# UniBwTAS/continuous_clustering

Hardware: AMD Instinct MI355X
Metric: Mpoints/s clustered (64-beam streams) (higher is better)
Workload: dtype f32

## Files before the change

continuous_clustering_amd/csrc/cc_assoc3.h:

```cpp
#pragma once

constexpr int A3_REC = 8;
constexpr int A3_THREADS = 256;
constexpr int A3_PSTAGE = 8;
constexpr int A3_BIRTH = 8;

template<int RPL>
__device__ __forceinline__ void assoc3_stream(const Geometry& g, const cc_config& cfg, const Planes& P, StreamState* states, const int s, const int slot,
                                              const int limited)
{
    constexpr int G = RPL == 1 ? 8 : 4;
    constexpr int A2_LEAD = a2_lead(RPL), A2_STAGE = a2_stage(RPL);
    static_assert(WIN_COLS + A2_LEAD + 1 <= WIN2_COLS && A2_LEAD + G <= A2_STAGE && A2_LEAD < A2_INFO, "ring sizes");
    const int lane = lane_id();
    const int wave = uniform_i32((int) (threadIdx.x >> 6));
    const bool lwave = blockDim.x > 192;
    const int nthreads = (int) blockDim.x;
    StreamState* st = &states[s];
    if (st->error != 0 || st->batch[slot].seg_begin < 0 || st->assoc_mode != 0 || st->batch[slot].mode != 0 ||
        st->batch[slot].acp_next >= st->batch[slot].seg_end)
        return;
    AssocCtx c;
    c.p = stream_ptrs(P, g, s);
    const SP& p = c.p;
// ... 1297 lines not shown
                    }
                }
                wave_lds_fence();
            }

            A2_PH(3)
#ifdef CC_A2_STATS
            st_nunf += n_unf;
            st_sub++;
            st_check += cut == CUT_CHECK;
            st_live += cut == CUT_LIVE;
#endif
            int check_u = -1;
            if (cut == CUT_CHECK)
            {
                check_u = u1 - 1;
                u0 = u1;
            }
            else if (cut == CUT_LIVE)
            {
                const int u = u1;
                const long long gcu = gc + u;
                int lcu = lc0 + u;
                lcu = lcu >= RC ? lcu - RC : lcu;
                emit(CC_EV_GROUND_COLUMN, gcu, gcu, 0, 0, gcu);
                serial_cols++;
                wait_a(gcu + 1);
                if (err)
                    break;
                const int info_head = uniform_i32(lds_ld(&T.info_head[(int) (gcu & (A2_INFO - 1))]));
                park_a();
                if (err)
                    break;
                if (lane == 0)
                {
                    int nn = n_unf, e = 0, hd = info_head;
                    double LL = L;
                    long long MM = M;
                    assoc_column_live2<RPL>(c, cfg, g, T, s_win, lcu, gcu, (int) (first_unpub % RC), nn, LL, MM, hd, e, st);
                    T.bcast_i[0] = nn;
                    T.bcast_i[1] = e;
                    T.bcast_i[3] = hd;
                    T.bcast_d[0] = LL;
                    T.bcast_l[0] = MM;
                }
                wave_lds_fence();
                n_unf = uniform_i32(T.bcast_i[0]);
                const int hd = uniform_i32(T.bcast_i[3]);
                if (uniform_i32(T.bcast_i[1]) == CC_ERR_CAPACITY)
                {
                    err = CC_ERR_CAPACITY;
                    err_a = n_unf;
                }
                L = uniform_f64(T.bcast_d[0]);
                M = uniform_i64(T.bcast_l[0]);
                wave_lds_fence();
                if (err)
                    break;
                resume_a(gcu + 1, hd);
                check_u = u;
                u0 = u1 + 1;
                ids_stale = true;
            }
            else if (cut == CUT_GLOBAL)
            {
                to_global = true;
                gc += u1;
                break;
            }
            else
                u0 = gcount;
            if (check_u >= 0)
            {
                finish_and_publish(gc + check_u, lane_f64(v_minaz, check_u));
                verify |= killed;
            }
            if (lane == 0)
                lds_st(&T.b_done, gc + u0);
            A2_PH(4)
        }
        if (to_global || err)
            break;
        gc += gcount;
        lc0 += gcount;
        lc0 = lc0 >= RC ? lc0 - RC : lc0;
    }
    if (lane == 0)
        lds_st(&T.cmd, (int) A2_EXIT);
#ifdef CC_A2_STATS
    if (lane == 0)
    {
        st->dbg[8] += st_sub;
        st->dbg[9] += st_check;
        st->dbg[10] += __builtin_amdgcn_s_memtime() - st_t0;
        st->dbg[11] += st_live;
        st->dbg[12] += (unsigned long long) (gc - col_begin);
        st->dbg[13] += st_wait_g;
        st->dbg[14] += st_full;
        st->dbg[15] += st_kill;
        for (int i = 0; i < 5; i++)
            st->dbg[i] += st_ph[i];
    }
#endif

    {
        wave_lds_fence();
        for (int r = lane; r < n_unf; r += 64)
        {
            const int i = T.alist[r];
            const int cell = T.cell[i];
            p.ulist[r] = cell;
            p.t_pos[cell] = r;
            p.t_fin[cell] = __longlong_as_double((long long) T.fin[i]);
            p.t_width[cell] = (unsigned) (T.last[i] - T.gcol[i] + 1);
            p.t_pts[cell] = T.pts[i];
            p.t_uf[cell] = T.cell[T.uf[i]];
            p.t_cid[cell] = 0;
            p.t_finished[cell] = 0;
        }
    }
    if (lane == 0)
    {
        st->first_unpublished = first_unpub;
        st->batch[slot].pub_end = first_unpub;
        st->ring_start = ring_start;
        st->cluster_counter = cluster_counter;
        st->n_unfinished = n_unf;
        st->min_required = M;
        st->finish_lower_bound = L;
        st->last_round_min_az = last_min_az;
        st->cells_published = cells_published;
        st->clusters_finished = clusters_finished;
        st->exceed_one_rotation = exceed;
        st->serial_columns = serial_cols;
        st->stamp_alias_rounds = alias_rounds;
        st->batch[slot].acp_next = gc;
        st->n_events = n_events < g.event_capacity ? n_events : g.event_capacity;
        if (g.record_events && n_events > g.event_capacity && err == 0)
        {
            err = CC_ERR_CAPACITY;
            err_a = n_events;
        }
        if (to_global)
            st->assoc_mode = 1;
        if (err)
            raise_error(st, err, err_a, err_b);
    }
}

template<int RPL>
__global__ __launch_bounds__(A3_THREADS) void k_assoc3(Geometry g, cc_config cfg, Planes P, StreamState* states, int first_stream, int slot,
                                                       int limited, int count, int with_global)
{
    if (gridDim.x >= (unsigned) count)
    {
        if ((int) blockIdx.x < count)
        {
            assoc3_stream<RPL>(g, cfg, P, states, first_stream + (int) blockIdx.x, slot, limited);
            if (with_global && !limited)
            {
                __threadfence_block();
                __syncthreads();
                if (threadIdx.x < 64)
                    associate_stream<RPL>(g, cfg, P, states, first_stream + (int) blockIdx.x, slot);
            }
        }
        return;
    }
    __shared__ int s_work[A3_THREADS];
    __shared__ int s_nwork;
    if (threadIdx.x == 0)
        s_nwork = 0;
    __syncthreads();
    for (int base = 0; base < count; base += (int) (gridDim.x * blockDim.x))
    {
        const int i = base + (int) threadIdx.x * (int) gridDim.x + (int) blockIdx.x;
        if (i < count)
        {
            const StreamState* st = &states[first_stream + i];
            if (st->error == 0 && st->batch[slot].seg_begin >= 0 && st->batch[slot].acp_next < st->batch[slot].seg_end)
                s_work[atomicAdd(&s_nwork, 1)] = i;
        }
        __syncthreads();
        const int nw = s_nwork;
        for (int k = 0; k < nw; k++)
        {
            assoc3_stream<RPL>(g, cfg, P, states, first_stream + s_work[k], slot, limited);
            __threadfence_block();
            __syncthreads();
            if (with_global && !limited)
            {
                if (threadIdx.x < 64)
                    associate_stream<RPL>(g, cfg, P, states, first_stream + s_work[k], slot);
                __syncthreads();
            }
        }
        if (threadIdx.x == 0)
            s_nwork = 0;
        __syncthreads();
    }
}
```

continuous_clustering_amd/csrc/cc_engine.hip:

```cpp
#include <hip/hip_runtime.h>

#include <algorithm>
#include <chrono>
#include <cstdlib>
#include <cmath>
#include <cstdio>
#include <cstring>
#include <functional>
#include <limits>
#include <mutex>
#include <string>
#include <vector>

#include "cc_kernels.h"

#ifndef CC_LWAVE_MAX_STREAMS
#define CC_LWAVE_MAX_STREAMS 256
#endif

using namespace ccd;

struct cc_engine
{
    int device{0};
    Geometry g{};
    cc_config cfg{};
    Planes P{};
    StreamState* d_states{nullptr};
    int* d_remaining{nullptr};
    int* h_remaining{nullptr};
    int* d_bail_count{nullptr};
    int* h_bail_count{nullptr};
    int bail_seen{0}, bail_cooldown{0};
    int chronic_seen{0}, chronic_skip{0};
    bool chronic_probe{false};
    int assoc_sweep_blocks{2};
    int bail_cooldown_batches{4};
    bool capturing{false};
    cck::HostMirror capture_mirror{nullptr, nullptr, 0, nullptr, nullptr, nullptr, nullptr};
    int* d_par_left{nullptr};
    bool small_front{true};
    bool small_all{true};
    bool small_direct{true};
    int seg_small_max{63};
    bool fuse_front{true};
    int* h_par_left{nullptr};
    int insert_split_blocks{0};
    int insert_wide_max_streams{160};
    bool skip_idle_fallbacks{true};
    hipStream_t stream{nullptr};
    hipStream_t stream2{nullptr};
    hipStream_t stream3{nullptr};
    hipStream_t stream4{nullptr};
    hipStream_t stream6{nullptr};
    hipEvent_t ev_pubrdy[4]{};
    hipStream_t stream5{nullptr};
    hipEvent_t ev_ins[4]{}, ev_seg[4]{}, ev_assoc[4]{}, ev_segscan[4]{}, ev_prep[4]{};
    hipEvent_t ev_input{};
    int pipeline_depth{2};
    int prep_buf{0};
    std::vector<hipEvent_t> pev_pool;
    size_t pev_used{0};
    struct PrepPlanes
    {
        float *x, *y, *z, *dist, *incl, *incaz;
        int32_t* cir;
    } pp[2]{};
    uint64_t batch_seq{0};
    static constexpr int REL_RING = 8;
    uint64_t call_seq{0};
    uint64_t released_seq{0};
    hipEvent_t ev_rel[REL_RING]{};
    uint64_t rel_recorded[REL_RING]{};
    bool in_submit{false};
    bool cur_call_last{true};
    int check_input_lifetime{0};
    struct InputRec
    {
        uint64_t seq;
        const void *xyz, *inten, *pose;
        size_t b_xyz, b_int, b_pose;
        unsigned long long sum;
    };
    std::vector<InputRec> live_inputs;
    unsigned long long* d_input_sum{nullptr};
    unsigned long long* h_input_sum{nullptr};
    bool pipelined{false};
    bool allow_pipeline{true};
    bool host_prof{false};
    double hp_pre{0}, hp_gate{0}, hp_post{0}, hp_entry{0};
    long long hp_calls{0};
    bool parallel_insert_multi{true};
    bool parallel_insert{true};
    struct SmallGraph
    {
        int stream;
        int64_t n;
        int record;
        hipGraphExec_t exec;
    };
    std::vector<SmallGraph> small_graphs;
    unsigned char* h_small{nullptr};
    unsigned char* d_small{nullptr};
    unsigned long long* h_small_seq{nullptr};
    unsigned long long* d_small_seq{nullptr};
    unsigned long long small_seq_expected{0};
    unsigned long long small_tail_launches{0};
    long long* h_small_view_hdr{nullptr};
    char* h_small_view{nullptr};
    bool small_view_ok{false};
    int small_view_stream{-1};
    bool mirror_views{true};
    unsigned long long view_hits{0}, view_misses{0};
    bool resident_opt{false};
    bool res_running{false};
    cck::ResidentCtl* h_res_ctl{nullptr};
    int res_idle_ms{20};
    unsigned long long res_launches{0}, res_calls{0};
    StreamState* h_small_state{nullptr};
    cc_event* h_small_events{nullptr};
    bool allow_graphs{true};
    int scan_store_fin{-1};
    int scan_split{2};
    bool split_on{false};
    unsigned split_cols_seen{0}, split_rec_seen{0}, split_probe{0};
    int scan_packed{-1};
    int assoc_waves{3};
    bool assoc_batch{true};
    int assoc_rounds{0};
    bool assoc_waves_auto{true};
    bool assoc_pending[4]{false, false, false, false};
    std::vector<void*> allocations;
    std::function<int(const std::function<int()>*)> deferred_tail;
    int lazy_gate_max_streams{40};
    int lazy_gate_from_streams{80};
    bool lazy_ok{true};
    bool lazy_pending{false};
    const int* lazy_prev_left{nullptr};
    int lazy_miss{0};
    int lazy_clean{0};
    uint64_t lazy_batches{0}, lazy_redone{0};
    hipEvent_t ev_gate[4]{};
    int defer_tail_max_streams{96};
    bool slab_planning{false};
    size_t slab_bytes{0};
    std::vector<std::pair<void**, size_t>> slab_plan;
    std::string error;
    float* d_stage_xyz{nullptr};
    uint8_t* d_stage_int{nullptr};
    double* d_stage_pose{nullptr};
    int64_t stage_capacity{0};
    size_t prep_capacity{0};
    void* d_view{nullptr};
    size_t view_bytes{0};
    double* d_ego[4]{nullptr, nullptr, nullptr, nullptr};
    size_t ego_capacity{0};
    bool small_graphs_stale{false};
    bool idle{false};
    std::vector<StreamState> state_cache;
    std::vector<char> state_cached;
    char* d_gather{nullptr};
    size_t gather_bytes{0};
    char* h_view{nullptr};
    size_t h_view_bytes{0};
    std::vector<std::vector<cc_event>> pending_events;
    std::vector<std::vector<int64_t>> pending_links;
    const float* last_xyz{nullptr};
    const uint8_t* last_int{nullptr};
    const double* last_pose{nullptr};
    int64_t last_n{0};
    int64_t cur_ntotal{0}, cur_f0{0};
    int64_t sub_batch{0};
    bool input_on_engine_stream{false};
    int last_first{0}, last_count{0};
    bool batch_open{false};
    bool timing{false};
    int timing_every{1};
    uint64_t timing_pass{0};
    double prep_ahead_ms{0};
    std::vector<hipEvent_t> ev_pool;
    size_t ev_used{0};
    double kernel_ms[7]{0, 0, 0, 0, 0, 0, 0};
    uint64_t kernel_launches{0};
};

namespace
{

constexpr size_t CC_SLAB_ALIGN = 2u << 20;

#define CC_HIP_CHECK(e, call)                                                                                      \
    do                                                                                                             \
    {                                                                                                              \
        hipError_t _err = (call);                                                                                  \
        if (_err != hipSuccess)                                                                                    \
        {                                                                                                          \
            (e)->error = std::string(#call) + ": " + hipGetErrorString(_err);                                      \
            return CC_ERR_HIP;                                                                                     \
        }                                                                                                          \
    } while (0)

template<class T>
int alloc_plane(cc_engine* e, T** out, size_t count)
{
    if (e->slab_planning)
    {
        const size_t bytes = (count * sizeof(T) + CC_SLAB_ALIGN - 1) / CC_SLAB_ALIGN * CC_SLAB_ALIGN;
        e->slab_plan.push_back({(void**) out, e->slab_bytes});
        e->slab_bytes += bytes;
        return CC_OK;
    }
    void* p = nullptr;
    hipError_t err = hipMalloc(&p, count * sizeof(T));
    if (err != hipSuccess)
    {
        e->error = std::string("hipMalloc: ") + hipGetErrorString(err);
        return CC_ERR_HIP;
    }
    e->allocations.push_back(p);
    *out = (T*) p;
    return CC_OK;
}

int validate(cc_engine* e, const cc_config* cfg, int num_rows, int num_streams)
{
    if (!cfg || num_rows < 1 || num_rows > WAVE * MAX_ROWS_PER_LANE || num_streams < 1 || cfg->num_columns < 4 ||
        cfg->cluster_point_trees_every_nth_column < 1)
    {
        if (e)
            e->error = "invalid argument (num_rows must be 1..128, num_columns >= 4, every_nth_column >= 1)";
        return CC_ERR_INVALID_ARGUMENT;
    }
    return CC_OK;
}

void fill_geometry(cc_engine* e, int num_rows)
{
    Geometry& g = e->g;
    g.num_rows = num_rows;
    g.num_columns = e->cfg.num_columns;
    g.az_width = static_cast<float>((2 * M_PI)) / static_cast<float>(g.num_columns);
    g.ring_cols = g.num_columns * 10;
    g.cells = (int64_t) g.ring_cols * num_rows;
    g.max_distance_squared = e->cfg.max_distance * e->cfg.max_distance;
    g.limit_columns = 2 * g.num_columns;
    g.tab_tiles = g.ring_cols / 64 + 2;
    if (g.lds_tree_limit <= 0 || g.lds_tree_limit > TREE_SLOTS)
        g.lds_tree_limit = TREE_SLOTS;
    if (g.sl_cap <= 0 || g.sl_cap > cck::SL_CAP)
        g.sl_cap = cck::SL_CAP;
    if (g.scan_cap <= 0)
        g.scan_cap = cck::SCAN_CAP;
    g.scan_stores_fin = 0;
}

int free_all(cc_engine* e)
{
    for (void* p : e->allocations)
        (void) hipFree(p);
    e->allocations.clear();
    e->d_stage_xyz = nullptr;
    e->d_stage_int = nullptr;
    e->d_stage_pose = nullptr;
    e->stage_capacity = 0;
    e->d_view = nullptr;
    e->view_bytes = 0;
    e->prep_capacity = 0;
    e->ego_capacity = 0;
    e->d_gather = nullptr;
    e->gather_bytes = 0;
    e->d_small = nullptr;
    e->d_small_seq = nullptr;
    e->d_input_sum = nullptr;
    if (e->h_res_ctl)
        (void) hipHostFree(e->h_res_ctl);
    e->h_res_ctl = nullptr;
    if (e->h_small_view_hdr)
        (void) hipHostFree(e->h_small_view_hdr);
    if (e->h_small_view)
        (void) hipHostFree(e->h_small_view);
    e->h_small_view_hdr = nullptr;
    e->h_small_view = nullptr;
    e->small_view_ok = false;
    if (e->h_input_sum)
        (void) hipHostFree(e->h_input_sum);
    e->h_input_sum = nullptr;
    e->small_seq_expected = 0;
    if (e->h_small)
    {
        (void) hipHostFree(e->h_small);
        (void) hipHostFree(e->h_small_state);
        (void) hipHostFree(e->h_small_events);
        if (e->h_small_seq)
            (void) hipHostFree(e->h_small_seq);
        e->h_small_seq = nullptr;
        e->h_small = nullptr;
        e->h_small_state = nullptr;
        e->h_small_events = nullptr;
    }
    return CC_OK;
}

int allocate(cc_engine* e)
{
    const Geometry& g = e->g;
    const size_t S = (size_t) g.num_streams;
    const size_t C = S * (size_t) g.cells;
    const size_t L = S * (size_t) g.ring_cols;
    const size_t T = S * (size_t) g.tree_capacity;
    Planes& P = e->P;
    int rc = CC_OK;
    e->slab_planning = getenv("CC_NO_SLAB") == nullptr;
    e->slab_bytes = 0;
    e->slab_plan.clear();
#define A(field, count)                                \
    if ((rc = alloc_plane(e, &P.field, (count))) != 0) \
        return rc;
    A(dist, C) A(incl, C) A(incaz, C) A(gtag, C) A(src, C) A(inten, C);
    A(trig, L) A(colg, L) A(colminaz, L);
    A(ground, C) A(debug, C) A(ignored, C) A(root, C) A(id, C);
    A(t_fin, C) A(t_width, C) A(t_pts, C) A(t_uf, C) A(t_cid, C) A(t_pos, C) A(t_finished, C);
    A(ulist, T) A(ucomp, T) A(agg_fin, T) A(agg_min, T) A(agg_max, T) A(agg_pts, T) A(agg_cid, T) A(agg_first, T) A(agg_flag, T);
    A(events, S * (size_t) g.event_capacity);
    A(sc_parent, C) A(sc_nlinks, C) A(sc_links, C) A(sc_fin, C);
    A(sc_term, C) A(col_newfin, L) A(col_info, L) A(col_act, L) A(pk_meta, C) A(pk_fin, C) A(pk_lk, C);
    A(sg_x2, C) A(sg_uz, C) A(sg_w, C) A(sg_flags, C) A(sc_rec, C);
    A(curtab, S * (size_t) g.num_rows);
    A(tab_acc, S * (size_t) g.tab_tiles * (size_t) g.num_rows);
    A(par_off, S * (size_t) cck::IP_MAXF);
    A(tabc, (size_t) BATCH_SLOTS * S * (size_t) g.tab_tiles * (size_t) g.num_rows);
    A(sc_visits, C);
    A(link_log, S * (size_t) g.link_capacity);
    A(sl_ctl, S * 4) A(sl_cols, L);
    if ((rc = alloc_plane(e, (unsigned long long**) &P.sl_rec, S * (size_t) cck::SL_CAP * sizeof(cck::ScanLongRec) / sizeof(unsigned long long))) != 0)
        return rc;
#undef A
    if ((rc = alloc_plane(e, &e->d_states, S)) != 0)
        return rc;
    if ((rc = alloc_plane(e, &e->d_par_left, 16)) != 0)
        return rc;
    if ((rc = alloc_plane(e, &e->d_bail_count, 4)) != 0)
        return rc;
    if ((rc = alloc_plane(e, &e->d_remaining, 1)) != 0)
        return rc;
    const bool slab = e->slab_planning;
    if (e->slab_planning)
    {
        e->slab_planning = false;
        char* base = nullptr;
        if ((rc = alloc_plane(e, &base, e->slab_bytes)) != 0)
            return rc;
        for (auto& f : e->slab_plan)
            *f.first = base + f.second;
        e->slab_plan.clear();
    }
    (void) slab;
    CC_HIP_CHECK(e, hipMemset(e->d_bail_count, 0, 4 * sizeof(int)));
    CC_HIP_CHECK(e, hipMemset(e->d_par_left, 0, 16 * sizeof(int)));
    CC_HIP_CHECK(e, hipMemset(e->d_remaining, 0, sizeof(int)));
    return CC_OK;
}

int reset_state(cc_engine* e, bool keep_table)
{
    e->small_view_ok = false;
    std::fill(e->state_cached.begin(), e->state_cached.end(), 0);
    const Geometry& g = e->g;
    const size_t S = (size_t) g.num_streams;
    const size_t C = S * (size_t) g.cells;
    Planes& P = e->P;
    CC_HIP_CHECK(e, hipMemsetAsync(P.dist, 0xFF, C * sizeof(float), e->stream));
    CC_HIP_CHECK(e, hipMemsetAsync(P.incl, 0xFF, C * sizeof(float), e->stream));
    CC_HIP_CHECK(e, hipMemsetAsync(P.gtag, 0, C * sizeof(uint16_t), e->stream));
    CC_HIP_CHECK(e, hipMemsetAsync(P.id, 0, C * sizeof(uint32_t), e->stream));
    CC_HIP_CHECK(e, hipMemsetAsync(P.ground, CC_GP_UNKNOWN, C, e->stream));
    CC_HIP_CHECK(e, hipMemsetAsync(P.debug, CC_DBG_WHITE, C, e->stream));
    CC_HIP_CHECK(e, hipMemsetAsync(P.ignored, 0, C, e->stream));
    CC_HIP_CHECK(e, hipMemsetAsync(P.root, 0xFF, C * sizeof(int32_t), e->stream));
    CC_HIP_CHECK(e, hipMemsetAsync(P.tab_acc, 0, S * (size_t) g.tab_tiles * (size_t) g.num_rows * sizeof(unsigned long long), e->stream));
    CC_HIP_CHECK(e, hipMemsetAsync(P.sl_ctl, 0, S * 4 * sizeof(int32_t), e->stream));
    if (!keep_table)
        CC_HIP_CHECK(e, hipMemsetAsync(P.curtab, 0xFF, S * (size_t) g.num_rows * sizeof(float), e->stream));
    std::vector<StreamState> init(S);
    for (auto& st : init)
    {
        memset(&st, 0, sizeof(st));
        st.prev_rearmost = 0;
        st.prev_foremost = -1;
        st.first_unfinished = -1;
        st.ring_start = -1;
        st.ring_end = -1;
        st.first_column = -1;
        st.clear_done = -1;
        st.first_unpublished = -1;
        st.cluster_counter = 1;
        st.min_required = 0;
        st.finish_lower_bound = std::numeric_limits<double>::max();
        st.last_round_min_az = -1.0;
        st.overrun_col = std::numeric_limits<int64_t>::max();
        st.n_links = 0;
        for (auto& d : st.batch)
            d.seg_begin = d.seg_end = d.acp_next = d.pub_begin = d.pub_end = -1, d.mode = 0, d.fused = 0;
        st.assoc_mode = e->cfg.max_steps_in_row > WIN_COLS - 2 ? 1 : 0;
    }
    CC_HIP_CHECK(e, hipMemcpyAsync(e->d_states, init.data(), S * sizeof(StreamState), hipMemcpyHostToDevice, e->stream));
    CC_HIP_CHECK(e, hipStreamSynchronize(e->stream));
    for (auto& v : e->pending_events)
        v.clear();
    for (auto& v : e->pending_links)
        v.clear();
    e->batch_open = false;
    for (bool& b : e->assoc_pending)
        b = false;
    e->deferred_tail = nullptr;
    e->lazy_pending = false;
    e->lazy_prev_left = nullptr;
    e->lazy_miss = 0;
    e->lazy_clean = 0;
    e->lazy_ok = true;
    return CC_OK;
}

int ensure_prep(cc_engine* e, size_t points)
{
    if (e->prep_capacity >= points)
        return CC_OK;
    int rc;
    for (auto& q : e->pp)
        if ((rc = alloc_plane(e, &q.x, points)) || (rc = alloc_plane(e, &q.y, points)) || (rc = alloc_plane(e, &q.z, points)) ||
            (rc = alloc_plane(e, &q.dist, points)) || (rc = alloc_plane(e, &q.incl, points)) ||
            (rc = alloc_plane(e, &q.incaz, points)) || (rc = alloc_plane(e, &q.cir, points)))
            return rc;
    e->prep_capacity = points;
    e->small_graphs_stale = true;
    return CC_OK;
}

int take_timing_events(cc_engine* e, hipEvent_t* ev)
{
    for (int i = 0; i < 10; i++)
    {
        if (e->ev_used == e->ev_pool.size())
        {
            hipEvent_t x;
            CC_HIP_CHECK(e, hipEventCreate(&x));
            e->ev_pool.push_back(x);
        }
        ev[i] = e->ev_pool[e->ev_used++];
    }
    return CC_OK;
}

static Planes planes_with_prep(const cc_engine* e, int buf)
{
    Planes P = e->P;
    const auto& q = e->pp[buf];
    P.pp_x = q.x;
    P.pp_y = q.y;
    P.pp_z = q.z;
    P.pp_dist = q.dist;
    P.pp_incl = q.incl;
    P.pp_incaz = q.incaz;
    P.pp_cir = q.cir;
    return P;
}

int launch_prep(cc_engine* e, int count, int64_t n, const float* d_xyz, const double* d_pose, int buf, hipStream_t sp, int64_t n_total,
                int64_t f0, bool skip_inserted = false, int first_stream = 0)
{
    const size_t points = (size_t) count * (size_t) n * e->g.num_rows;
    int rcp = ensure_prep(e, points);
    if (rcp)
        return rcp;
    const Planes P = planes_with_prep(e, buf);
    const size_t per_stream = (size_t) n * e->g.num_rows;
    hipLaunchKernelGGL(cck::k_prep, dim3((unsigned) ((per_stream + cck::PREP_POINTS_PER_BLOCK - 1) / cck::PREP_POINTS_PER_BLOCK), (unsigned) count), dim3(256), 0, sp,
                       e->g, e->cfg, P,
                       d_xyz, d_pose, (long long) n, (long long) n_total, (long long) f0, skip_inserted ? (const StreamState*) e->d_states : nullptr,
                       first_stream);
    return CC_OK;
}

static int stop_resident(cc_engine* e)
{
    if (!e->res_running)
        return CC_OK;
    __atomic_store_n(&e->h_res_ctl->stop, 1ull, __ATOMIC_RELEASE);
    const hipError_t err = hipStreamSynchronize(e->stream);
    e->res_calls += __atomic_load_n(&e->h_res_ctl->calls, __ATOMIC_ACQUIRE);
    e->res_running = false;
    __atomic_store_n(&e->h_res_ctl->stop, 0ull, __ATOMIC_RELEASE);
    if (err != hipSuccess)
    {
        e->error = std::string("stopping the resident kernel: ") + hipGetErrorString(err);
        return CC_ERR_HIP;
// ... 397 lines not shown
            const size_t lds = cck::seg_scan_lds_bytes(g.num_rows);
            hipLaunchKernelGGL(cck::k_seg_scan, seg_grid, dim3(64), lds, sb, g, e->cfg, Pt, e->d_states, first_stream, slot);
        }
        if (sc != sb)
        {
            CC_HIP_CHECK(e, hipEventRecord(e->ev_segscan[slot], sb));
            CC_HIP_CHECK(e, hipStreamWaitEvent(sc, e->ev_segscan[slot], 0));
        }
        CC_MARK(sc);
        bool batch_assoc = e->assoc_batch && e->cfg.cluster_point_trees_every_nth_column == 1;
        if (batch_assoc && e->assoc_rounds == 0 && e->h_bail_count && !e->capturing && count >= 8)
        {
            const int seen_now = *e->h_bail_count;
            if (e->chronic_skip > 0)
            {
                e->chronic_skip--;
                e->bail_seen = seen_now;
                batch_assoc = false;
                if (e->chronic_skip == 0)
                    e->bail_cooldown = e->bail_cooldown_batches > 2 ? e->bail_cooldown_batches : 2;
            }
            else if ((seen_now - e->chronic_seen) * 4 >= count && e->chronic_probe)
                e->chronic_skip = 8;
            e->chronic_probe = batch_assoc;
            e->chronic_seen = seen_now;
        }
        int adaptive_rounds = 1;
        if (e->assoc_rounds == 0 && e->h_bail_count && !e->capturing)
        {
            const int seen = *e->h_bail_count;
            if (seen != e->bail_seen)
            {
                e->bail_seen = seen;
                e->bail_cooldown = e->bail_cooldown_batches;
            }
            if (e->bail_cooldown > 0)
            {
                e->bail_cooldown--;
                adaptive_rounds = 3;
            }
        }
        Geometry gs = g;
        gs.scan_stores_fin = (!small_front && !(batch_assoc && e->assoc_rounds == 0 && adaptive_rounds == 1)) ? 1 : 0;
        if (e->scan_store_fin >= 0 && !small_front)
            gs.scan_stores_fin = e->scan_store_fin;
        const dim3 scan_grid((unsigned) count, cck::SCAN_BLOCKS);
        bool use_split = false;
        if (small_front)
            ;
        else if ([&]() -> bool
                 {
                     const bool packed_default = e->scan_packed == 1 || (e->scan_packed < 0 && (rpl > 1 || count > 192));
                     use_split = false;
                     if (g.mirror_fields || e->scan_split == 0)
                         return packed_default;
                     if (e->scan_split == 1 || !e->h_bail_count || e->capturing)
                     {
                         use_split = packed_default && e->scan_split == 1;
                         return packed_default;
                     }
                     const unsigned vis = (unsigned) e->h_bail_count[1], cols = (unsigned) e->h_bail_count[2];
                     const unsigned dc = cols - e->split_cols_seen, dv = vis - e->split_rec_seen;
                     if (dc >= 1024u)
                     {
                         const double rate = (double) dv / ((double) dc * (double) rpl);
                         e->split_on = e->split_on ? rate > 20.0 : rate > 40.0;
                         e->split_cols_seen = cols, e->split_rec_seen = vis;
                     }
                     const bool probe = (e->split_probe++ & 31u) == 0u;
                     const bool promote = !packed_default && e->scan_packed < 0 && rpl == 1 && count >= 48;
                     use_split = (e->split_on || probe) && (packed_default || promote);
                     return packed_default || (promote && use_split);
                 }())
        {
            const bool split = use_split;
            if (split)
            {
                const dim3 long_grid((unsigned) count, cck::SCAN_LONG_BLOCKS), epi_grid((unsigned) count, cck::SCAN_EPI_BLOCKS);
                if (rpl == 1)
                {
                    hipLaunchKernelGGL((cck::k_scan2<1, false, true>), scan_grid, dim3(64), 0, sc, gs, e->cfg, e->P, e->d_states, first_stream, slot);
                    hipLaunchKernelGGL(cck::k_scan2_long<1>, long_grid, dim3(64), 0, sc, g, e->cfg, e->P, e->d_states, first_stream, slot, e->d_bail_count);
                    hipLaunchKernelGGL(cck::k_scan2_epi<1>, epi_grid, dim3(64), 0, sc, g, e->cfg, e->P, e->d_states, first_stream, slot, e->d_bail_count);
                }
                else
                {
                    hipLaunchKernelGGL((cck::k_scan2<2, false, true>), scan_grid, dim3(64), 0, sc, gs, e->cfg, e->P, e->d_states, first_stream, slot);
                    hipLaunchKernelGGL(cck::k_scan2_long<2>, long_grid, dim3(64), 0, sc, g, e->cfg, e->P, e->d_states, first_stream, slot, e->d_bail_count);
                    hipLaunchKernelGGL(cck::k_scan2_epi<2>, epi_grid, dim3(64), 0, sc, g, e->cfg, e->P, e->d_states, first_stream, slot, e->d_bail_count);
                }
            }
            else if (rpl == 1 && !g.mirror_fields)
                hipLaunchKernelGGL((cck::k_scan2<1, false>), scan_grid, dim3(64), 0, sc, gs, e->cfg, e->P, e->d_states, first_stream, slot);
            else if (rpl == 1)
                hipLaunchKernelGGL((cck::k_scan2<1, true>), scan_grid, dim3(64), 0, sc, gs, e->cfg, e->P, e->d_states, first_stream, slot);
            else if (!g.mirror_fields)
                hipLaunchKernelGGL((cck::k_scan2<2, false>), scan_grid, dim3(64), 0, sc, gs, e->cfg, e->P, e->d_states, first_stream, slot);
            else
                hipLaunchKernelGGL((cck::k_scan2<2, true>), scan_grid, dim3(64), 0, sc, gs, e->cfg, e->P, e->d_states, first_stream, slot);
        }
        else if (rpl == 1 && !g.mirror_fields)
            hipLaunchKernelGGL((cck::k_scan<1, false>), scan_grid, dim3(64), 0, sc, gs, e->cfg, e->P, e->d_states, first_stream, slot);
        else if (rpl == 1)
            hipLaunchKernelGGL((cck::k_scan<1, true>), scan_grid, dim3(64), 0, sc, gs, e->cfg, e->P, e->d_states, first_stream, slot);
        else if (!g.mirror_fields)
            hipLaunchKernelGGL((cck::k_scan<2, false>), scan_grid, dim3(64), 0, sc, gs, e->cfg, e->P, e->d_states, first_stream, slot);
        else
            hipLaunchKernelGGL((cck::k_scan<2, true>), scan_grid, dim3(64), 0, sc, gs, e->cfg, e->P, e->d_states, first_stream, slot);
        CC_MARK(sc);
        if (sc != sa)
        {
            CC_HIP_CHECK(e, hipEventRecord(e->ev_seg[slot], sc));
            CC_HIP_CHECK(e, hipStreamWaitEvent(sa, e->ev_seg[slot], 0));
        }
        CC_MARK(sa);
        auto launch_assocb = [&]()
        {
            if (rpl == 1)
                hipLaunchKernelGGL(cck::k_assocb<1>, dim3(count), dim3(cck::AB_THREADS), 0, sa, g, e->cfg, e->P, e->d_states, first_stream, slot,
                                   e->d_bail_count);
            else
                hipLaunchKernelGGL(cck::k_assocb<2>, dim3(count), dim3(cck::AB_THREADS), 0, sa, g, e->cfg, e->P, e->d_states, first_stream, slot,
                                   e->d_bail_count);
        };
        bool marked7 = false;
        bool global_done = false;
        const bool small_tail = small_front && e->capture_mirror.state != nullptr && batch_assoc && e->assoc_waves >= 2 && rpl == 1 &&
                                e->cfg.cluster_point_trees_every_nth_column == 1;
        if (small_tail)
        {
            launch_assocb();
            CC_MARK(sa);
            marked7 = true;
            hipLaunchKernelGGL(cck::k_small_tail<1>, dim3(1), dim3(cck::A3_THREADS), 0, sa, g, e->cfg, e->P, e->d_states, first_stream, slot, e->capture_mirror);
            global_done = true;
        }
        else if (e->assoc_waves >= 2 && e->cfg.cluster_point_trees_every_nth_column == 1)
        {
            const bool lwave = e->assoc_waves == 4 || (e->assoc_waves_auto && count <= CC_LWAVE_MAX_STREAMS);
            const dim3 block(lwave ? cck::A3_THREADS : 192);
            const int rounds = batch_assoc ? (e->assoc_rounds > 0 ? e->assoc_rounds : adaptive_rounds) : 1;
            for (int r = 0; r < rounds; r++)
            {
                if (batch_assoc)
                {
                    launch_assocb();
                    if (r == 0)
                    {
                        CC_MARK(sa);
                        marked7 = true;
                    }
                }
                const int limited = r + 1 < rounds ? 1 : 0;
                const int blocks = (batch_assoc && e->assoc_rounds == 0 && adaptive_rounds == 1 && !e->capturing) ? (count < e->assoc_sweep_blocks ? count : e->assoc_sweep_blocks) : count;
                if (rpl == 1)
                    hipLaunchKernelGGL(cck::k_assoc3<1>, dim3(blocks), block, 0, sa, gs, e->cfg, e->P, e->d_states, first_stream, slot, limited, count, 1);
                else
                    hipLaunchKernelGGL(cck::k_assoc3<2>, dim3(blocks), block, 0, sa, gs, e->cfg, e->P, e->d_states, first_stream, slot, limited, count, 1);
                global_done = limited == 0;
            }
        }
        else
        {
            if (batch_assoc)
            {
                launch_assocb();
                CC_MARK(sa);
                marked7 = true;
            }
            if (rpl == 1)
                hipLaunchKernelGGL(cck::k_assoc_lds<1>, dim3(count), dim3(64), 0, sa, gs, e->cfg, e->P, e->d_states, first_stream, slot);
            else
                hipLaunchKernelGGL(cck::k_assoc_lds<2>, dim3(count), dim3(64), 0, sa, gs, e->cfg, e->P, e->d_states, first_stream, slot);
        }
        if (!marked7)
            CC_MARK(sa);
        if (global_done)
            ;
        else if (rpl == 1)
            hipLaunchKernelGGL(cck::k_associate<1>, dim3(count), dim3(64), 0, sa, g, e->cfg, e->P, e->d_states, first_stream, slot);
        else
            hipLaunchKernelGGL(cck::k_associate<2>, dim3(count), dim3(64), 0, sa, g, e->cfg, e->P, e->d_states, first_stream, slot);
        CC_MARK(sa);
        if (batch_assoc && !gate && !gate2 && e->h_bail_count && !e->capturing)
            CC_HIP_CHECK(e, hipMemcpyAsync(e->h_bail_count, e->d_bail_count, 3 * sizeof(int), hipMemcpyDeviceToHost, sa));
        hipStream_t spub = si != sa ? e->stream6 : sa;
        if (spub != sa)
        {
            CC_HIP_CHECK(e, hipEventRecord(e->ev_pubrdy[slot], sa));
            CC_HIP_CHECK(e, hipStreamWaitEvent(spub, e->ev_pubrdy[slot], 0));
        }
        if (!small_tail)
            hipLaunchKernelGGL(cck::k_publish, dim3((unsigned) count, cck::PUBLISH_BLOCKS), dim3(64), 0, spub, g, e->P, e->d_states, first_stream,
                               slot, e->capture_mirror);
        CC_MARK(spub);
        if (si != sa)
        {
            CC_HIP_CHECK(e, hipEventRecord(e->ev_assoc[slot], spub));
            e->assoc_pending[slot] = true;
            if (rel_seq)
            {
                CC_HIP_CHECK(e, hipEventRecord(e->ev_rel[rel_seq % cc_engine::REL_RING], spub));
                e->rel_recorded[rel_seq % cc_engine::REL_RING] = rel_seq;
            }
        }
        CC_HIP_CHECK(e, hipGetLastError());
        if (e->host_prof && hp_gated)
        {
            e->hp_post += std::chrono::duration<double>(std::chrono::steady_clock::now() - hp_t1).count();
            e->hp_calls++;
        }
        return CC_OK;
    };
#undef CC_MARK
    if (lazy_registered)
    {
        const long long my_ntotal = e->cur_ntotal, my_f0 = e->cur_f0;
        const int my_prep_buf = e->prep_buf;
        e->deferred_tail = [=](const std::function<int()>* redo) mutable -> int
        {
            CC_HIP_CHECK(e, hipEventSynchronize(e->ev_gate[slot]));
            const bool fb = gate_h_left[0] != 0, seg = gate_h_left[1] != 0;
            if (!fb && !seg)
            {
                e->lazy_miss = 0;
                return tail(0, 0, 1);
            }
            if (++e->lazy_miss >= 2)
                e->lazy_ok = false;
            const long long keep_ntotal = e->cur_ntotal, keep_f0 = e->cur_f0;
            const int keep_buf = e->prep_buf;
            e->cur_ntotal = my_ntotal, e->cur_f0 = my_f0, e->prep_buf = my_prep_buf;
            int rc = tail(fb ? 1 : 0, seg ? 1 : 0, 0);
            if (!rc && hipStreamSynchronize(si) != hipSuccess)
                rc = CC_ERR_HIP;
            if (!rc && *e->h_remaining != 0)
                rc = finish_batch(e);
            e->cur_ntotal = keep_ntotal, e->cur_f0 = keep_f0, e->prep_buf = keep_buf;
            if (!rc && redo)
            {
                e->lazy_redone++;
                rc = (*redo)();
            }
            return rc;
        };
        e->lazy_pending = true;
        e->lazy_prev_left = gate_left;
        return CC_OK;
    }
    if (defer)
    {
        e->deferred_tail = [tail](const std::function<int()>*) mutable -> int { return tail(-1, -1, -1); };
        return CC_OK;
    }
    return tail(-1, -1, -1);
}

__global__ void k_clear_remaining(int* remaining)
{
    *remaining = 0;
}

__global__ void k_clear_events(StreamState* states, int first_stream, int count)
{
    int i = blockIdx.x * blockDim.x + threadIdx.x;
    if (i < count)
    {
        states[first_stream + i].n_events = 0;
        states[first_stream + i].n_links = 0;
    }
}

int collect_events(cc_engine* e, int first_stream, int count);
int collect_links(cc_engine* e, int stream, const StreamState& st);

int resolve_timing(cc_engine* e)
{
    static const int from[7] = {0, 1, 3, 4, 6, 7, 8};
    for (size_t i = 0; i + 9 < e->ev_used; i += 10)
    {
        for (int k = 0; k < 7; k++)
        {
            float ms = 0.f;
            CC_HIP_CHECK(e, hipEventElapsedTime(&ms, e->ev_pool[i + from[k]], e->ev_pool[i + from[k] + 1]));
            e->kernel_ms[k] += ms;
        }
        e->kernel_launches++;
    }
    for (size_t i = 0; i + 1 < e->pev_used; i += 2)
    {
        float ms = 0.f;
        CC_HIP_CHECK(e, hipEventElapsedTime(&ms, e->pev_pool[i], e->pev_pool[i + 1]));
        e->prep_ahead_ms += ms;
    }
    e->pev_used = 0;
    e->ev_used = 0;
    return CC_OK;
}

int sync_all(cc_engine* e)
{
    {
        int rcf = flush_deferred(e);
        if (rcf)
            return rcf;
    }
    if (e->idle)
        return CC_OK;
    {
        int rcs = stop_resident(e);
        if (rcs)
// ... 1893 lines not shown
```

continuous_clustering_amd/csrc/cc_k_assoc_global.h:

```cpp
#pragma once

constexpr int LINK_SLOTS_V1 = 8;

struct AssocCtx
{
    SP p;
    int R, NC, RC;
    float az_width, maxd2;
    int max_steps_in_row, max_steps_in_column, stop_enabled, stop_min_steps;
};

__device__ __forceinline__ int uf_find(int32_t* uf, int a)
{
    while (true)
    {
        const int pa = ld_agent(&uf[a]);
        if (pa == a)
            return a;
        const int gp = ld_agent(&uf[pa]);
        if (gp != pa)
            __hip_atomic_store(&uf[a], gp, __ATOMIC_RELAXED, __HIP_MEMORY_SCOPE_AGENT);
        a = pa;
    }
}
// ... 4 lines not shown
    {
        a = uf_find(uf, a);
        b = uf_find(uf, b);
        if (a == b)
            return;
        if (a < b)
        {
            const int t = a;
            a = b;
            b = t;
        }
        if (atomicCAS(&uf[a], a, b) == a)
            return;
    }
}

__device__ __forceinline__ void tree_init(const SP& p, int cell, double fin)
{
    p.t_fin[cell] = fin;
    p.t_width[cell] = 1;
    p.t_pts[cell] = 1;
    p.t_uf[cell] = cell;
    p.t_cid[cell] = 0;
    p.t_finished[cell] = 0;
}

struct NoLinkVisitor
{
    __device__ __forceinline__ void operator()(int) const {}
};
template<bool LIVE, bool CODE = false, bool REC = false, class ON_LINK = NoLinkVisitor>
__device__ __forceinline__ void scan_point(const AssocCtx& c, const int lc, const long long gc, const int row, const int first_local,
                                           const float mad, const double pcaz, int& p_root, int& parent, int* links, int& nlinks,
                                           bool& overflow, const int max_links = LINK_SLOTS_V1, int* visits = nullptr, StreamState* st = nullptr,
                                           const Geometry* geo = nullptr, int* reach = nullptr, const ON_LINK& on_link = ON_LINK())
{
    const SP& p = c.p;
    const int R = c.R;
    const int pi = lc * R + row;
    const float4 me = p.sc_rec[pi];
    const float pincl = me.w, px = me.x, py = me.y, pz = me.z;
    int needed = f2i_x86(__builtin_ceilf(mad / c.az_width));
    needed = needed < c.max_steps_in_row ? needed : c.max_steps_in_row;
    int oc = lc;
    bool rooted = LIVE ? (p_root != -1) : false;
    for (int sb = 0; sb <= needed; sb++)
    {
        for (int dir = -1; dir <= 1; dir += 2)
        {
            if (dir == 1 && sb == 0)
                continue;
            int sv = (dir == 1 || sb == 0) ? 1 : 0;
            int orow = (dir == 1 || sb == 0) ? row + dir : row;
            while (orow >= 0 && orow < R && sv <= c.max_steps_in_column)
            {
                const int oi = oc * R + orow;
                if (visits)
                    ++*visits;
                if (reach)
                    *reach = sb;
                const float4 orec = p.sc_rec[oi];
                unsigned char oign = 0;
                if (REC)
                    oign = p.ignored[oi];
                const float oincl = orec.w;
                if (ccm::absf(oincl - pincl) > mad)
                    break;
                if (REC ? !oign : !p.ignored[oi])
                {
                    bool consider = true;
                    int oroot = -1;
                    if (LIVE)
                    {
                        oroot = p.root[oi];
                        consider = (p_root >= 0 && p_root / R == 0) || oroot != p_root;
                    }
                    if (consider)
                    {
                        const float dx = px - orec.x, dy = py - orec.y, dz = pz - orec.z;
                        if (dx * dx + dy * dy + dz * dz < c.maxd2)
                        {
                            if (LIVE)
                            {
                                if (p_root == -1)
                                {
                                    const long long rg = p.colg[oroot / R];
                                    const uint32_t nw = (uint32_t) (gc - rg + 1);
                                    if (nw <= (uint32_t) c.NC && !p.t_finished[oroot])
                                    {
                                        p_root = oroot;
                                        parent = (sb << 8) | orow;
                                        p.t_width[oroot] = nw;
                                        const double cand = pcaz + (double) mad;
                                        const double cur = ld_agent(&p.t_fin[oroot]);
                                        if (cand > cur)
                                            __hip_atomic_store(&p.t_fin[oroot], cand, __ATOMIC_RELAXED, __HIP_MEMORY_SCOPE_AGENT);
                                        atomicAdd(&p.t_pts[oroot], 1u);
                                    }
                                }
                                else
                                {
                                    if (!p.t_finished[p_root] && !p.t_finished[oroot] && p_root != oroot)
                                    {
                                        if (geo)
                                            log_link(*geo, st, p.link_log, p_root, oroot);
                                        uf_union(p.t_uf, p_root, oroot);
                                    }
                                }
                            }
                            else
                            {
                                const int cand = CODE ? ((sb << 8) | orow) : oi;
                                if (!rooted)
                                {
                                    parent = cand;
                                    rooted = true;
                                }
                                else
                                {
                                    on_link(cand);
                                    if (nlinks < max_links)
                                        links[nlinks++] = cand;
                                    else
                                        overflow = true;
                                }
                            }
                        }
                    }
                }
                if (LIVE)
                    rooted = p_root != -1;
                if (rooted && c.stop_enabled && sv >= c.stop_min_steps)
                    break;
                orow += dir;
                sv++;
            }
        }
        if (rooted && c.stop_enabled && sb >= c.stop_min_steps)
            break;
        if (oc == first_local)
            break;
        oc--;
        if (oc < 0)
            oc += c.RC;
    }
}

__device__ __forceinline__ void assoc_wave_sync()
{
    __builtin_amdgcn_fence(__ATOMIC_RELEASE, "workgroup");
    __builtin_amdgcn_fence(__ATOMIC_ACQUIRE, "workgroup");
}

template<int RPL>
__device__ __forceinline__ void associate_stream(const Geometry& g, const cc_config& cfg, const Planes& P, StreamState* states, const int s, const int slot)
{
    const int lane = lane_id();
    StreamState* st = &states[s];
    if (st->error != 0 || st->batch[slot].seg_begin < 0 || (st->assoc_mode == 0 && st->batch[slot].mode == 0) ||
        st->batch[slot].acp_next >= st->batch[slot].seg_end)
        return;
    AssocCtx c;
    c.p = stream_ptrs(P, g, s);
    const SP& p = c.p;
    const int R = c.R = g.num_rows;
    const int NC = c.NC = g.num_columns;
    const int RC = c.RC = g.ring_cols;
    c.az_width = g.az_width;
    c.maxd2 = g.max_distance_squared;
    c.max_steps_in_row = cfg.max_steps_in_row;
    c.max_steps_in_column = cfg.max_steps_in_column;
    c.stop_enabled = cfg.stop_after_association_enabled;
    c.stop_min_steps = cfg.stop_after_association_min_steps;
    const int nth = cfg.cluster_point_trees_every_nth_column;

    __shared__ int s_parent[WAVE * MAX_ROWS_PER_LANE];
    __shared__ int s_links[WAVE * MAX_ROWS_PER_LANE][LINK_SLOTS_V1];
    __shared__ int s_bcast[4];
    __shared__ double s_bd[2];
    __shared__ long long s_bl[2];

    long long first_unpub = st->first_unpublished, ring_start = st->ring_start;
    if (lane == 0 && st->batch[slot].pub_begin < 0)
        st->batch[slot].pub_begin = first_unpub;
    unsigned long long cluster_counter = st->cluster_counter;
    int n_unf = st->n_unfinished;
    long long M = st->min_required;
    double L = st->finish_lower_bound;
    double last_min_az = st->last_round_min_az;
    unsigned long long cells_published = st->cells_published, clusters_finished = st->clusters_finished;
    unsigned long long exceed = st->exceed_one_rotation, serial_cols = st->serial_columns, alias_rounds = st->stamp_alias_rounds;
    int n_events = st->n_events;
    const long long col_end = st->batch[slot].seg_end;
    int err = 0;
    long long err_a = 0, err_b = 0;

    auto emit = [&](int type, long long a, long long b, unsigned cc, unsigned dd, long long column)
    {
        if (!g.record_events)
            return;
        if (lane == 0)
        {
            if (n_events < g.event_capacity)
            {
                cc_event e;
                e.type = type;
                e.stream = s;
                e.a = a;
                e.b = b;
                e.c = cc;
                e.d = dd;
                e.column = column;
                p.events[n_events] = e;
            }
        }
        n_events++;
    };

    for (long long gc = st->batch[slot].acp_next; gc < col_end && err == 0; gc++)
    {
        const int lc = (int) (gc % RC);
        const int first_local = (int) (first_unpub % RC);
        const CazBase cb = caz_base_of_column(gc, g.num_columns);
        emit(CC_EV_GROUND_COLUMN, gc, gc, 0, 0, gc);

        float mad[RPL];
        double pcaz[RPL];
        bool active[RPL];
        int parent[RPL], nlinks[RPL];
        bool overflow = false;
#pragma unroll
        for (int k = 0; k < RPL; k++)
        {
            const int row = k * 64 + lane;
            active[k] = false;
            parent[k] = -1;
            nlinks[k] = 0;
            mad[k] = 0.f;
            pcaz[k] = 0.;
            if (row < R)
            {
                const int ci = lc * R + row;
                if (!p.ignored[ci])
                {
                    active[k] = true;
                    mad[k] = ccm::asinf_exact(cfg.max_distance / p.dist[ci]);
                    pcaz[k] = cell_caz(cb, p.incaz[ci]);
                    int dummy_root = -1, vis = 0;
                    scan_point<false>(c, lc, gc, row, first_local, mad[k], pcaz[k], dummy_root, parent[k], s_links[row], nlinks[k],
                                      overflow, LINK_SLOTS_V1, &vis);
                    if (g.mirror_fields)
                        p.sc_visits[ci] = sat_u16(vis);
                }
                s_parent[row] = active[k] ? parent[k] : -2;
                {
                    int code = active[k] ? -1 : -2;
                    if (parent[k] >= 0)
                    {
                        int back = lc - parent[k] / R;
                        back = back < 0 ? back + RC : back;
                        code = (back << 8) | (parent[k] % R);
                    }
                    p.sc_parent[ci] = (int16_t) code;
                    if (!active[k] && g.mirror_fields)
                        p.sc_visits[ci] = 0;
                }
            }
        }
        assoc_wave_sync();
        int rootc[RPL];
        bool refused = overflow;
#pragma unroll
        for (int k = 0; k < RPL; k++)
        {
            const int row = k * 64 + lane;
            rootc[k] = -1;
            if (active[k])
            {
                if (parent[k] < 0)
                    rootc[k] = lc * R + row;
                else
                {
                    int r = parent[k];
                    while (true)
                    {
                        if (r / R != lc)
                        {
                            r = p.root[r];
                            break;
                        }
                        const int pr = s_parent[r - lc * R];
                        if (pr < 0)
                            break;
                        r = pr;
                    }
                    rootc[k] = r;
                    if (r < 0)
                        refused = true;
                    else
                    {
                        const long long rg = p.colg[r / R];
                        const uint32_t nw = (uint32_t) (gc - rg + 1);
                        if (nw > (uint32_t) NC || p.t_finished[r])
                            refused = true;
                    }
                }
            }
        }
        const bool column_serial = __any(refused);

        if (!column_serial)
        {
#pragma unroll
            for (int k = 0; k < RPL; k++)
            {
                const int row = k * 64 + lane;
                const bool is_new = active[k] && parent[k] < 0;
                const unsigned long long mask = __ballot(is_new);
                const int cnt = __popcll(mask);
                if (n_unf + cnt > g.tree_capacity)
                {
                    err = CC_ERR_CAPACITY;
                    err_a = n_unf + cnt;
                    break;
                }
                if (row < R)
                    p.root[lc * R + row] = active[k] ? rootc[k] : -1;
                if (is_new)
                {
                    const int cell = lc * R + row;
                    const int pos = n_unf + __popcll(mask & lanes_below());
                    const double fin = pcaz[k] + (double) mad[k];
                    tree_init(p, cell, fin);
// ... 137 lines not shown
            {
                const int t = p.ulist[i];
                const int rep = uf_find(p.t_uf, t);
                const int j = p.t_pos[rep];
                p.ucomp[i] = j;
                const long long tg = p.colg[t / R];
                atomicMax(&p.agg_fin[j], (unsigned long long) __double_as_longlong(ld_agent(&p.t_fin[t])));
                atomicMin(&p.agg_min[j], tg);
                atomicMax(&p.agg_max[j], tg + (long long) p.t_width[t]);
                atomicAdd(&p.agg_pts[j], ld_agent(&p.t_pts[t]));
                atomicMin(&p.agg_first[j], i);
            }
            assoc_wave_sync();
            int exceed_local = 0;
            for (int i = lane; i < n_unf; i += 64)
            {
                if (p.ucomp[i] == i)
                {
                    const double fin = __longlong_as_double((long long) ld_agent(&p.agg_fin[i]));
                    const bool unfinished = fin > min_az;
                    const bool exceeds = (ld_agent(&p.agg_max[i]) - ld_agent(&p.agg_min[i])) >= NC;
                    if (exceeds)
                        exceed_local++;
                    p.agg_flag[i] = (!unfinished || exceeds) ? 1 : 0;
                }
            }
            for (int o = 32; o > 0; o >>= 1)
                exceed_local += __shfl_xor(exceed_local, o);
            exceed += exceed_local;
            assoc_wave_sync();
            int last_first = -1;
            while (true)
            {
                int best = 0x7fffffff;
                for (int i = lane; i < n_unf; i += 64)
                    if (p.ucomp[i] == i && p.agg_flag[i] && ld_agent(&p.agg_pts[i]) > 5u)
                    {
                        const int fi = ld_agent(&p.agg_first[i]);
                        if (fi > last_first && fi < best)
                            best = fi;
                    }
                best = wave_min_i32(best);
                if (best == 0x7fffffff)
                    break;
                const int j = p.ucomp[best];
                const unsigned cid = (unsigned) cluster_counter;
                if (lane == 0)
                    p.agg_cid[j] = cid;
                emit(CC_EV_CLUSTER, ld_agent(&p.agg_min[j]), ld_agent(&p.agg_max[j]) - 1, cid, ld_agent(&p.agg_pts[j]), gc);
                cluster_counter++;
                clusters_finished++;
                last_first = best;
            }
            assoc_wave_sync();
            long long min_all = 0x7fffffffffffffffll, min_surv = 0x7fffffffffffffffll;
            double L_new = 1.7976931348623157e308;
            int out = 0;
            for (int base = 0; base < n_unf; base += 64)
            {
                const int i = base + lane;
                bool surv = false;
                int t = -1;
                if (i < n_unf)
                {
                    t = p.ulist[i];
                    const int j = p.ucomp[i];
                    const long long tg = p.colg[t / R];
                    min_all = tg < min_all ? tg : min_all;
                    if (p.agg_flag[j])
                    {
                        p.t_finished[t] = 1;
                        p.t_cid[t] = p.agg_cid[j];
                    }
                    else
                    {
                        surv = true;
                        min_surv = tg < min_surv ? tg : min_surv;
                        if (j == i)
                        {
                            const double fin = __longlong_as_double((long long) ld_agent(&p.agg_fin[i]));
                            L_new = fin < L_new ? fin : L_new;
                        }
                    }
                }
                const unsigned long long mask = __ballot(surv);
                if (surv)
                {
                    const int np = out + __popcll(mask & lanes_below());
                    p.ulist[np] = t;
                    p.t_pos[t] = np;
                }
                out += __popcll(mask);
            }
            min_all = wave_min_i64(min_all);
            min_surv = wave_min_i64(min_surv);
            L = wave_min_f64(L_new);
            M_c = min_all;
            M = min_surv;
            n_unf = out;
            assoc_wave_sync();
        }
        last_min_az = min_az;

        if (M_c < first_unpub)
        {
            err = CC_ERR_BOOKKEEPING;
            err_a = M_c;
            err_b = first_unpub;
            break;
        }
        const long long old_unpub = first_unpub, old_ring = ring_start;
        first_unpub = M_c;
        ring_start = first_unpub - NC > 0 ? first_unpub - NC : 0;
        emit(CC_EV_PUBLISH_COLUMNS, old_unpub, first_unpub - 1, 0, 0, gc);
        cells_published += (unsigned long long) (first_unpub - old_unpub) * (unsigned long long) R;
        (void) old_ring;
    }

    if (lane == 0)
    {
        st->first_unpublished = first_unpub;
        st->batch[slot].pub_end = first_unpub;
        st->ring_start = ring_start;
        st->cluster_counter = cluster_counter;
        st->n_unfinished = n_unf;
        st->min_required = M;
        st->finish_lower_bound = L;
        st->last_round_min_az = last_min_az;
        st->cells_published = cells_published;
        st->clusters_finished = clusters_finished;
        st->exceed_one_rotation = exceed;
        st->serial_columns = serial_cols;
        st->stamp_alias_rounds = alias_rounds;
        st->batch[slot].acp_next = col_end;
        if (err == 0)
            st->assoc_mode = (cfg.max_steps_in_row > WIN_COLS - 2 || n_unf * 2 > g.lds_tree_limit) ? 1 : 0;
        st->n_events = n_events < g.event_capacity ? n_events : g.event_capacity;
        if (g.record_events && n_events > g.event_capacity && err == 0)
        {
            err = CC_ERR_CAPACITY;
            err_a = n_events;
        }
        if (err)
            raise_error(st, err, err_a, err_b);
    }
}

template<int RPL>
__global__ __launch_bounds__(64) void k_associate(Geometry g, cc_config cfg, Planes P, StreamState* states, int first_stream, int slot)
{
    associate_stream<RPL>(g, cfg, P, states, first_stream + (int) blockIdx.x, slot);
}


template<int RPL, bool MIRROR>
__device__ __forceinline__ void scan_column_epilogue(const SP& p, const int R, const int lc, const int lane, const int (&parent)[RPL],
                                                     const int (&nlinks)[RPL], const double (&fin)[RPL], const unsigned long long (&packed)[RPL],
                                                     int reach)
{
    int t[RPL];
#pragma unroll
    for (int k = 0; k < RPL; k++)
    {
        const int row = k * 64 + lane;
        const bool same_col = parent[k] >= 0 && (parent[k] >> 8) == 0;
        t[k] = same_col ? (parent[k] & 0xff) : row;
    }
    for (int it = 0; it < 7; it++)
    {
        int nt[RPL];
        bool changed = false;
#pragma unroll
        for (int k = 0; k < RPL; k++)
        {
            const int src = t[k];
            const int lo = __shfl(t[0], src & 63);
            const int hi = RPL > 1 ? __shfl(t[RPL - 1], src & 63) : lo;
            nt[k] = src < 64 ? lo : hi;
            changed |= nt[k] != t[k];
        }
#pragma unroll
        for (int k = 0; k < RPL; k++)
            t[k] = nt[k];
        if (!__any(changed))
            break;
    }
    int cnt_new = 0, mine[RPL];
    int max_delta = 0;
    int flags = 0;
    int n_act = 0;
    double newfin = 1.7976931348623157e308;
#pragma unroll
    for (int k = 0; k < RPL; k++)
    {
        n_act |= __popcll(__ballot(parent[k] >= -1)) << (8 * k);
        const bool is_new = parent[k] == -1;
        const unsigned long long mask = __ballot(is_new);
        const int newidx = cnt_new + __popcll(mask & lanes_below());
        cnt_new += __popcll(mask);
        mine[k] = is_new ? newidx : (parent[k] >= 0 ? parent[k] : -1);
        if (is_new && fin[k] < newfin)
            newfin = fin[k];
        if (parent[k] >= 0)
        {
            int d = parent[k] >> 8;
            const int nl = nlinks[k] == 255 ? LINK_SLOTS : nlinks[k];
            for (int j = 0; j < nl; j++)
            {
                const int dj = (int) ((packed[k] >> (16 * j + 8)) & 0xff);
                d = dj > d ? dj : d;
            }
            max_delta = d > max_delta ? d : max_delta;
        }
        if (nlinks[k] == 255)
            flags |= 1;
        else if (nlinks[k] > 0)
            flags |= 2;
    }
#pragma unroll
    for (int k = 0; k < RPL; k++)
    {
        const int row = k * 64 + lane;
        const int src = t[k];
        const int lo = __shfl(mine[0], src & 63);
        const int hi = RPL > 1 ? __shfl(mine[RPL - 1], src & 63) : lo;
        const int term = parent[k] < -1 ? -1 : (src < 64 ? lo : hi);
        if (row < R)
            p.sc_term[lc * R + row] = (int16_t) term;
        const unsigned long long actm = __ballot(parent[k] >= -1);
        if (parent[k] >= -1)
        {
            const int j = (k > 0 ? (n_act & 0xff) : 0) + __popcll(actm & lanes_below());
            const unsigned nlc = nlinks[k] == 255 ? 7u : (unsigned) nlinks[k];
            p.pk_meta[lc * R + j] = ((unsigned) term & 0xffffu) | ((unsigned) row << 16) | (nlc << 23) | (parent[k] == -1 ? 1u << 26 : 0u);
            p.pk_fin[lc * R + j] = fin[k];
            if (nlinks[k] > 0)
                p.pk_lk[lc * R + j] = packed[k];
        }
        else if (row < R)
            p.root[lc * R + row] = -1;
    }
    max_delta = -wave_min_i32(-max_delta);
    if (MIRROR)
        reach = -wave_min_i32(-reach);
    flags = (__any(flags & 1) ? 1 : 0) | (__any(flags & 2) ? 2 : 0);
    if (cnt_new > 0)
        newfin = wave_min_f64(newfin);
    if (lane == 0)
    {
        p.col_newfin[lc] = newfin;
        p.col_info[lc] = cnt_new | (flags << 8) | (max_delta << 16) | ((MIRROR ? reach : 0) << 24);
        p.col_act[lc] = (uint16_t) n_act;
    }
}
```

Measured before the change: 17970.

## Replace assoc3 sweep path with single-wave global-association rest kernel

The sweep case (few blocks handling the streams still left after batch association) no longer runs full 256-thread assoc3 blocks over a work list. It now launches a new 64-thread kernel that ballots for the remaining streams, forces them into global association mode, and runs associate_stream using per-stream scratch in global memory instead of LDS. The sweep block count rises from 2 to 4, and k_assoc3 is simplified to one block per stream. This aims to cut the cost of the leftover-stream sweep, but scratch in global memory adds memory latency, and switching the mode may change which path processes those streams.

```diff
diff --git a/continuous_clustering_amd/csrc/cc_assoc3.h b/continuous_clustering_amd/csrc/cc_assoc3.h
--- a/continuous_clustering_amd/csrc/cc_assoc3.h
+++ b/continuous_clustering_amd/csrc/cc_assoc3.h
@@ -1473,51 +1473,15 @@
 __global__ __launch_bounds__(A3_THREADS) void k_assoc3(Geometry g, cc_config cfg, Planes P, StreamState* states, int first_stream, int slot,
                                                        int limited, int count, int with_global)
 {
-    if (gridDim.x >= (unsigned) count)
-    {
-        if ((int) blockIdx.x < count)
-        {
-            assoc3_stream<RPL>(g, cfg, P, states, first_stream + (int) blockIdx.x, slot, limited);
-            if (with_global && !limited)
-            {
-                __threadfence_block();
-                __syncthreads();
-                if (threadIdx.x < 64)
-                    associate_stream<RPL>(g, cfg, P, states, first_stream + (int) blockIdx.x, slot);
-            }
-        }
-        return;
-    }
-    __shared__ int s_work[A3_THREADS];
-    __shared__ int s_nwork;
-    if (threadIdx.x == 0)
-        s_nwork = 0;
-    __syncthreads();
-    for (int base = 0; base < count; base += (int) (gridDim.x * blockDim.x))
-    {
-        const int i = base + (int) threadIdx.x * (int) gridDim.x + (int) blockIdx.x;
-        if (i < count)
-        {
-            const StreamState* st = &states[first_stream + i];
-            if (st->error == 0 && st->batch[slot].seg_begin >= 0 && st->batch[slot].acp_next < st->batch[slot].seg_end)
-                s_work[atomicAdd(&s_nwork, 1)] = i;
-        }
-        __syncthreads();
-        const int nw = s_nwork;
-        for (int k = 0; k < nw; k++)
-        {
-            assoc3_stream<RPL>(g, cfg, P, states, first_stream + s_work[k], slot, limited);
+    if ((int) blockIdx.x < count)
+    {
+        assoc3_stream<RPL>(g, cfg, P, states, first_stream + (int) blockIdx.x, slot, limited);
+        if (with_global && !limited)
+        {
             __threadfence_block();
             __syncthreads();
-            if (with_global && !limited)
-            {
-                if (threadIdx.x < 64)
-                    associate_stream<RPL>(g, cfg, P, states, first_stream + s_work[k], slot);
-                __syncthreads();
-            }
-        }
-        if (threadIdx.x == 0)
-            s_nwork = 0;
-        __syncthreads();
+            if (threadIdx.x < 64)
+                associate_stream<RPL>(g, cfg, P, states, first_stream + (int) blockIdx.x, slot);
+        }
     }
 }
diff --git a/continuous_clustering_amd/csrc/cc_engine.hip b/continuous_clustering_amd/csrc/cc_engine.hip
--- a/continuous_clustering_amd/csrc/cc_engine.hip
+++ b/continuous_clustering_amd/csrc/cc_engine.hip
@@ -30,11 +30,12 @@
     int* d_remaining{nullptr};
     int* h_remaining{nullptr};
     int* d_bail_count{nullptr};
+    cck::AssocScratch* d_assoc_scratch{nullptr};
     int* h_bail_count{nullptr};
     int bail_seen{0}, bail_cooldown{0};
     int chronic_seen{0}, chronic_skip{0};
     bool chronic_probe{false};
-    int assoc_sweep_blocks{2};
+    int assoc_sweep_blocks{4};
     int bail_cooldown_batches{4};
     bool capturing{false};
     cck::HostMirror capture_mirror{nullptr, nullptr, 0, nullptr, nullptr, nullptr, nullptr};
@@ -341,6 +342,8 @@
         return rc;
     if ((rc = alloc_plane(e, &e->d_bail_count, 4)) != 0)
         return rc;
+    if ((rc = alloc_plane(e, &e->d_assoc_scratch, S)) != 0)
+        return rc;
     if ((rc = alloc_plane(e, &e->d_remaining, 1)) != 0)
         return rc;
     const bool slab = e->slab_planning;
@@ -1044,11 +1047,20 @@
                     }
                 }
                 const int limited = r + 1 < rounds ? 1 : 0;
-                const int blocks = (batch_assoc && e->assoc_rounds == 0 && adaptive_rounds == 1 && !e->capturing) ? (count < e->assoc_sweep_blocks ? count : e->assoc_sweep_blocks) : count;
-                if (rpl == 1)
-                    hipLaunchKernelGGL(cck::k_assoc3<1>, dim3(blocks), block, 0, sa, gs, e->cfg, e->P, e->d_states, first_stream, slot, limited, count, 1);
+                if (batch_assoc && e->assoc_rounds == 0 && adaptive_rounds == 1 && !e->capturing)
+                {
+                    const int blocks = count < e->assoc_sweep_blocks ? count : e->assoc_sweep_blocks;
+                    if (rpl == 1)
+                        hipLaunchKernelGGL(cck::k_assoc_rest<1>, dim3(blocks), dim3(64), 0, sa, g, e->cfg, e->P, e->d_states, first_stream, slot, count,
+                                           e->d_assoc_scratch);
+                    else
+                        hipLaunchKernelGGL(cck::k_assoc_rest<2>, dim3(blocks), dim3(64), 0, sa, g, e->cfg, e->P, e->d_states, first_stream, slot, count,
+                                           e->d_assoc_scratch);
+                }
+                else if (rpl == 1)
+                    hipLaunchKernelGGL(cck::k_assoc3<1>, dim3(count), block, 0, sa, gs, e->cfg, e->P, e->d_states, first_stream, slot, limited, count, 1);
                 else
-                    hipLaunchKernelGGL(cck::k_assoc3<2>, dim3(blocks), block, 0, sa, gs, e->cfg, e->P, e->d_states, first_stream, slot, limited, count, 1);
+                    hipLaunchKernelGGL(cck::k_assoc3<2>, dim3(count), block, 0, sa, gs, e->cfg, e->P, e->d_states, first_stream, slot, limited, count, 1);
                 global_done = limited == 0;
             }
         }
diff --git a/continuous_clustering_amd/csrc/cc_k_assoc_global.h b/continuous_clustering_amd/csrc/cc_k_assoc_global.h
--- a/continuous_clustering_amd/csrc/cc_k_assoc_global.h
+++ b/continuous_clustering_amd/csrc/cc_k_assoc_global.h
@@ -180,8 +180,18 @@
     __builtin_amdgcn_fence(__ATOMIC_ACQUIRE, "workgroup");
 }
 
-template<int RPL>
-__device__ __forceinline__ void associate_stream(const Geometry& g, const cc_config& cfg, const Planes& P, StreamState* states, const int s, const int slot)
+struct AssocScratch
+{
+    int parent[WAVE * MAX_ROWS_PER_LANE];
+    int links[WAVE * MAX_ROWS_PER_LANE][LINK_SLOTS_V1];
+    int bcast[4];
+    double bd[2];
+    long long bl[2];
+};
+
+template<int RPL, bool GLOBAL_SCRATCH = false>
+__device__ __forceinline__ void associate_stream(const Geometry& g, const cc_config& cfg, const Planes& P, StreamState* states, const int s, const int slot,
+                                                 AssocScratch* scratch = nullptr)
 {
     const int lane = lane_id();
     StreamState* st = &states[s];
@@ -202,11 +212,19 @@
     c.stop_min_steps = cfg.stop_after_association_min_steps;
     const int nth = cfg.cluster_point_trees_every_nth_column;
 
-    __shared__ int s_parent[WAVE * MAX_ROWS_PER_LANE];
-    __shared__ int s_links[WAVE * MAX_ROWS_PER_LANE][LINK_SLOTS_V1];
-    __shared__ int s_bcast[4];
-    __shared__ double s_bd[2];
-    __shared__ long long s_bl[2];
+    AssocScratch* sw;
+    if constexpr (GLOBAL_SCRATCH)
+        sw = scratch + s;
+    else
+    {
+        __shared__ AssocScratch lw;
+        sw = &lw;
+    }
+    int* const s_parent = sw->parent;
+    int(*const s_links)[LINK_SLOTS_V1] = sw->links;
+    int* const s_bcast = sw->bcast;
+    double* const s_bd = sw->bd;
+    long long* const s_bl = sw->bl;
 
     long long first_unpub = st->first_unpublished, ring_start = st->ring_start;
     if (lane == 0 && st->batch[slot].pub_begin < 0)
@@ -650,6 +668,42 @@
     associate_stream<RPL>(g, cfg, P, states, first_stream + (int) blockIdx.x, slot);
 }
 
+template<int RPL>
+__global__ __launch_bounds__(64) void k_assoc_rest(Geometry g, cc_config cfg, Planes P, StreamState* states, int first_stream, int slot, int count,
+                                                   AssocScratch* scratch)
+{
+    const int lane = lane_id();
+    const int nb = (int) gridDim.x;
+    for (int base = 0; base < count; base += nb * WAVE)
+    {
+        const int i = base + lane * nb + (int) blockIdx.x;
+        bool left = false;
+        if (i < count)
+        {
+            const StreamState* st = &states[first_stream + i];
+            left = st->error == 0 && st->batch[slot].seg_begin >= 0 && st->batch[slot].acp_next < st->batch[slot].seg_end;
+        }
+        unsigned long long m = __ballot(left);
+        while (m)
+        {
+            const int k = __ffsll((long long) m) - 1;
+            m &= m - 1ull;
+            const int s = first_stream + base + k * nb + (int) blockIdx.x;
+            StreamState* st = &states[s];
+            if (lane == 0 && st->assoc_mode == 0 && st->batch[slot].mode == 0)
+            {
+                if (st->batch[slot].pub_begin < 0)
+                    st->batch[slot].pub_begin = st->first_unpublished;
+                st->batch[slot].pub_end = st->first_unpublished;
+                st->assoc_mode = 1;
+            }
+            __threadfence();
+            associate_stream<RPL, true>(g, cfg, P, states, s, slot, scratch);
+            __threadfence();
+        }
+    }
+}
+
 
 template<int RPL, bool MIRROR>
 __device__ __forceinline__ void scan_column_epilogue(const SP& p, const int R, const int lc, const int lane, const int (&parent)[RPL],
```

Result: slower. 17750, median of 2 (-1.2%).
